# daisy9542/yolo-puncture

Hardware: AMD Instinct MI355X
Metric: images/sec (higher is better)
Workload: dtype bf16

## Files before the change

### include/yolop.h

```cpp
#ifndef YOLOP_H
#define YOLOP_H

#include <stddef.h>
#include <stdint.h>

#ifdef __cplusplus
extern "C" {
#endif

#define YP_OK 0
#define YP_ERR_ARG -1
#define YP_ERR_STATE -2
#define YP_ERR_HIP -3
#define YP_ERR_WEIGHT -4

#define YP_BF16 0
#define YP_F32 1

#define YP_TASK_DETECT 0
#define YP_TASK_SEGMENT 1

#define YP_NM 32
#define YP_MAX_MASKS 480
#define YP_ID_MASKS_FRAMES_BUDGET (1ull << 30)
// ... 124 lines not shown
int yp_tensor_read(yp_engine* e, int i, float* host_out);

int yp_profile(yp_engine* e, const uint8_t* in_dev, int B, int H, int W, float* det_out, int32_t* idx_out,
               float* coeff_out, float* ms_out, int iters, void* stream);

int yp_set_nms(yp_engine* e, float conf, float iou);

int yp_set_attention_form(yp_engine* e, int form);

int yp_set_autotune(yp_engine* e, int enable);

int yp_tuning_export(const yp_engine* e, int32_t* cfg_out, int cap);
int yp_tuning_import(yp_engine* e, int B, int H, int W, const int32_t* cfg, int n);

int yp_debug_force_conv_cfg(int cfg);
int yp_debug_op_cfg(const yp_engine* e, int i, int* cfg);
int yp_debug_last_store_form(void);
int yp_debug_max_workgroups(int n);
int yp_debug_conv_families(int* base, int* num_cfgs, int cap);
int yp_debug_ablation(int v);
int yp_debug_head_clocks(uint64_t* out8);
int yp_debug_attention(const void* qkv_dev, void* o_dev, int dtype, int B, int N, int nh, int kd, int hd, int q_stride, int q_coff, int o_stride,
                       int o_coff, int wgs, int* kernel_out, void* stream);
int yp_debug_attention_form(const void* qkv_dev, void* o_dev, int dtype, int B, int N, int nh, int kd, int hd, int q_stride, int q_coff, int o_stride,
                            int o_coff, int wgs, int form, int* kernel_out, void* stream);
int yp_debug_conv_s2(const void* x_dev, const void* w_dev, const float* bias_dev, const void* res_dev, void* y_dev, int out_f32, int B, int H,
                     int W, int Cin, int Cout, int silu, int cfg, int lds_weights, int64_t* lds_out, char* kernel_out, int kernel_cap,
                     void* stream);
int yp_debug_topk_anchors(const uint32_t* const mk_dev[3], int B, const int hw[3][2], int k, int32_t* sel_out_dev, uint32_t* thr_out_dev, void* stream);
int yp_debug_head_branch_clocks(uint64_t* out8);
int yp_debug_head_winners(yp_engine* e, int32_t* sel_host, float* box_host, float* coeff_host);
int yp_debug_contour_clocks(uint64_t* out12);
int yp_debug_pwsp_clocks(uint64_t* out32);

int yp_tuning_source(const yp_engine* e);

int yp_debug_host_selftest(yp_engine* e);
int yp_debug_graph_info(const yp_engine* e, int64_t* out6);
int yp_debug_head_positions(yp_engine* e, int64_t* out6);
int yp_debug_marker(void* stream);

int yp_set_graph(yp_engine* e, int enable);

#ifdef __cplusplus
}
#endif
#endif
```

### yolo-puncture_amd/csrc/common.h

```cpp
#pragma once
#include <hip/hip_runtime.h>
#include <stdint.h>
#include <atomic>
#include <cstdlib>
#include <string>
#include <vector>

namespace yp {

enum DType { DT_BF16 = 0, DT_F32 = 1 };
enum Act { ACT_NONE = 0, ACT_SILU = 1, ACT_RELU = 2 };

enum OpKind {
    OP_STEM = 0,
    OP_CONV = 1,
    OP_DWCONV = 2,
    OP_POOL5 = 3,
    OP_UPSAMPLE = 4,
    OP_ATTN = 5,
    OP_HEAD = 6,
    OP_CONVT = 7,
    OP_AMAX = 9,
    OP_POOL3 = 8,
};
// ... 319 lines not shown
hipError_t launch_anchor_max_level(const float* cls, int B, int HW, int nc, unsigned* out, hipStream_t st);

struct DwPwParams {
    const void* x; int x_stride, x_coff; int B, H, W, C; size_t x_bytes;
    const void* w_dw; const float* b_dw; int act_dw;
    const void* w_pw; int Kpad; size_t wpw_bytes; const float* b_pw; int act_pw;
    void* y; int y_stride, y_coff; size_t y_bytes; int Cout; int out_f32;
    unsigned long long* clk;
    int wide;
    const void* w3; int Kpad3; size_t w3_bytes; const float* b3; int C3;
    float* y3; int y3_stride, y3_coff; size_t y3_bytes;
    unsigned* keys;
};
bool dwpw_stream_valid(const DwPwParams& p);
hipError_t launch_dwpw_stream(const DwPwParams& p, hipStream_t st);
struct PwSpParams {
    const void* x; int x_stride, x_coff; size_t x_bytes; int B, H, W, K;
    const void* w1; const float* bias1; int act1, Kpad1, C1; size_t w1_bytes;
    void* y1; int y1_stride, y1_coff;
    const void* res1; int res1_stride, res1_coff;
    int sp;
    int sp_c0, Csp;
    const void* wd; const float* biasd; int actd;
    const void* res; int res_stride, res_coff;
    void* y2; int y2_stride, y2_coff;
    int dbg;
    int wide;
};
bool pwsp_valid(const PwSpParams& p);
const char* pwsp_kernel_name(const PwSpParams& p);
constexpr int PWSP_CFG = 1000;
hipError_t launch_pwsp(const PwSpParams& p, hipStream_t st);
hipError_t pwsp_read_clocks(unsigned long long* out32);

struct ClsOutParams {
    const void* x; int x_stride, x_coff; size_t x_bytes;
    int M, K, nc;
    const void* w; int Kpad; size_t w_bytes; const float* bias;
    float* y; int y_stride, y_coff;
    unsigned* keys;
};
bool cls_out_valid(const ClsOutParams& p);
const char* cls_out_kernel_name(const ClsOutParams& p);
hipError_t launch_cls_out(const ClsOutParams& p, hipStream_t st);

bool conv_dwpw_valid(const DwPwParams& p);
const char* conv_dwpw_kernel_name(const DwPwParams& p);
hipError_t launch_conv_dwpw(const DwPwParams& p, hipStream_t st);

struct MaskParams {
    const void* proto; int Hp, Wp;
    const float* coeff; const float* boxes; int n;
    int oh, ow;
    int t, l, ch, cw;
    float bsx, bsy;
    int crop_before;
    uint8_t* masks; int64_t* ids; int32_t* kept; int32_t* area;
    int suppress_small, min_area;
    int rh, rw;
};
hipError_t launch_masks(const MaskParams& p, int dtype, hipStream_t st);
size_t masks_workspace_bytes(const MaskParams& p);
struct MaskFramesParams {
    MaskParams p;
    const int32_t* fidx; int k;
    size_t proto_stride; long coeff_stride;
// ... 39 lines not shown
```

### yolo-puncture_amd/csrc/engine.hip

```cpp
#include "../../include/yolop.h"
#include "common.h"
#include <algorithm>
#include <array>
#include <chrono>

#include <cmath>
#include <cstdarg>
#include <cstdio>
#include <cstring>
#include <cstdlib>
#include <dlfcn.h>
#include <fcntl.h>
#include <fstream>
#include <map>
#include <sstream>
#include <memory>

using namespace yp;

static thread_local char g_err[512] = "";
static int fail(int code, const char* fmt, ...) {
    va_list ap;
    va_start(ap, fmt);
    vsnprintf(g_err, sizeof(g_err), fmt, ap);
// ... 2427 lines not shown
    if (!e->allocated) return fail(YP_ERR_STATE, "no forward has run yet");
    const Op* h = nullptr;
    for (const Op& o : e->ops) if (o.kind == OP_HEAD) h = &o;
    if (!h || !(h->sparse_box || h->sparse_cf) || !e->sp_ws) return 0;
    HIPCHK(hipSetDevice(e->device));
    HIPCHK(hipDeviceSynchronize());
    const SparseWs ws = sparse_ws_layout(*e);
    const char* base = (const char*)e->sp_ws;
    int pc[8];
    HIPCHK(hipMemcpy(pc, base + ws.pcount, sizeof(pc), hipMemcpyDeviceToHost));
    std::vector<int> wc((size_t)e->pB * 3);
    HIPCHK(hipMemcpy(wc.data(), base + ws.wcount, wc.size() * 4, hipMemcpyDeviceToHost));
    for (int l = 0; l < 3; ++l) {
        out6[l] = std::min(pc[4 + l], ws.plist_cap[l]);
        for (int b = 0; b < e->pB; ++b) out6[3 + l] += wc[(size_t)b * 3 + l];
    }
    return 1;
}

__global__ void op_marker_kernel(int* sink) { if (sink) *sink = 0; }
int yp_debug_marker(void* stream) {
    hipLaunchKernelGGL(op_marker_kernel, dim3(1), dim3(1), 0, (hipStream_t)stream, (int*)nullptr);
    HIPCHK(hipGetLastError());
    return YP_OK;
}

int yp_debug_pwsp_clocks(uint64_t* out32) {
    if (!out32) return fail(YP_ERR_ARG, "yp_debug_pwsp_clocks: null output");
    HIPCHK(hipDeviceSynchronize());
    HIPCHK(pwsp_read_clocks((unsigned long long*)out32));
    return YP_OK;
}

int yp_debug_contour_clocks(uint64_t* out12) {
    if (!out12) return fail(YP_ERR_ARG, "yp_debug_contour_clocks: null output");
    HIPCHK(hipDeviceSynchronize());
    HIPCHK(contour_read_clocks((unsigned long long*)out12));
    return YP_OK;
}

int yp_debug_ablation(int v) {
    conv_set_debug_ablation(v);
    return 0;
}

int yp_debug_force_conv_cfg(int cfg) {
    conv_dma_force_cfg(cfg);
    return conv_dma_family.num_cfgs;
}

int yp_debug_last_store_form(void) {
    store_form_watched().store(true);
    return last_store_form().exchange(-1);
}

int yp_debug_max_workgroups(int n) { return debug_max_workgroups_ref().exchange(n > 0 ? n : 0); }

int yp_debug_op_cfg(const yp_engine* e, int i, int* cfg) {
    if (!e || i < 0 || i >= (int)e->ops.size() || !cfg) return fail(YP_ERR_ARG, "bad argument");
    *cfg = op_launch_cfg(*e, e->ops[i]);
    return YP_OK;
}

int yp_debug_conv_families(int* base, int* num_cfgs, int cap) {
    for (int f = 0; f < kNumConvFamilies && f < cap; ++f) {
        if (base) base[f] = kConvFamilies[f]->base;
// ... 377 lines not shown
```

### yolo-puncture_amd/csrc/pwsp.hip

```cpp
#include "common.h"
#include <cstdlib>
#include <algorithm>

namespace yp {

typedef __attribute__((ext_vector_type(4))) unsigned u32x4;

__device__ unsigned long long g_ps_clk[32];
#define PS_STAMP(i) do { if (blockIdx.x == 0 && tid == 0) g_ps_clk[i] = __builtin_readcyclecounter(); } while (0)
hipError_t pwsp_read_clocks(unsigned long long* out32) { return hipMemcpyFromSymbol(out32, HIP_SYMBOL(g_ps_clk), 32 * sizeof(unsigned long long)); }

constexpr int PS_MF = 2;
constexpr int PS_NW = 16;
constexpr int PS_NT = PS_NW * 64;

template <int NS, int SP>
__global__ __launch_bounds__(PS_NT) void pwsp_kernel(const PwSpParams p) {
    constexpr int FN = NS / 16;
    constexpr int BK = 64, NSLOT = 3;
    constexpr int W_INSTR = NS / 8;
    constexpr int SLOT = W_INSTR * 1024;
    constexpr int KS = SP == 1 ? 3 : SP == 2 ? 7 : 1, PAD = KS / 2;
    constexpr int PIX = SP == 3 ? NS * 2 : NS * 2 + 8;
    constexpr int DW_NP = NS / 2, DW_G = PS_NT / DW_NP;
    constexpr int DW_PH = NS == 64 ? 5 : 3, DW_PW = 3;
    static_assert(SP != 3 || NS == 32, "the pool form keeps 64-byte pixel rows");

    extern __shared__ __attribute__((aligned(1024))) unsigned char smem[];
    unsigned char* const dump = smem + NSLOT * SLOT;
    unsigned char* const img = smem + NSLOT * SLOT + 1024;

    const int tid = threadIdx.x, lane = tid & 63;
    const int wave = __builtin_amdgcn_readfirstlane(tid >> 6);
    const int fr = lane & 15, fc = lane >> 4;
    const int HW = p.H * p.W;
    const int nsl = p.C1 / NS;
    const bool wide = SP == 0 && p.wide != 0;

    int b, sl;
    {
        const int bid = blockIdx.x, nwg = gridDim.x;
        if ((p.B & 7) == 0) { const int xcd = bid & 7, j = bid >> 3; b = (j / nsl) * 8 + xcd; sl = j % nsl; }
        else { b = bid / nsl; sl = bid % nsl; }
        (void)nwg;
    }
    PS_STAMP(0);
    const int n0 = sl * NS;
    const bool spatial = SP != 0 && n0 >= p.sp_c0 && n0 + NS <= p.sp_c0 + p.Csp;
    const int nk = (p.Kpad1 + BK - 1) / BK;
    const __amdgpu_buffer_rsrc_t wrs = __builtin_amdgcn_make_buffer_rsrc((void*)p.w1, 0, (int)p.w1_bytes, 0x00020000);

    const int dgx = (p.W + DW_PW - 1) / DW_PW, dgy = (p.H + DW_PH - 1) / DW_PH;
    const int IW = (SP == 1 || SP == 2) ? dgx * DW_PW + 2 * PAD : p.W, IH = (SP == 1 || SP == 2) ? dgy * DW_PH + 2 * PAD : p.H;
    constexpr int PXS = 256 * 128;
    unsigned char* const wring = smem;
    unsigned char* const pxa = img;
    unsigned char* const pxb = img + 2 * PXS;
    const int nmf = (HW + 15) >> 4;
    const __amdgpu_buffer_rsrc_t xrs = __builtin_amdgcn_make_buffer_rsrc((void*)p.x, 0, (int)p.x_bytes, 0x00020000);
    unsigned pa_off[2], pb_off[2];
    int p_kc[2], w_kc;
#pragma unroll
    for (int j = 0; j < 2; ++j) {
        const int row = (wave * 2 + j) * 8 + (lane >> 3);
        const int c = (lane & 7) ^ ((row >> 1) & 7);
        p_kc[j] = c * 8;
        pa_off[j] = (row < HW && row < 256) ? (unsigned)((b * HW + row) * p.x_stride + p.x_coff + c * 8) * 2u : kBufferOOB;
        pb_off[j] = (row + 256 < HW) ? (unsigned)((b * HW + row + 256) * p.x_stride + p.x_coff + c * 8) * 2u : kBufferOOB;
    }
    unsigned wconst;
    {
        const int s_ = wave * 64 + lane;
        const int row = s_ >> 3, pc = s_ & 7;
        const int c = pc ^ ((row >> 1) & 7);
        w_kc = c * 8;
        wconst = (wave < W_INSTR) ? (unsigned)(((n0 + weight_row_channel(row, wide)) * p.Kpad1 + c * 8) * 2) : kBufferOOB;
    }
    auto kbyte = [&](int kt) { return (unsigned)(kt * BK) * 2u; };
    auto issue_A = [&](int kt) {
        const bool live = kt < nk;
        const unsigned kb = kbyte(kt);
        __builtin_amdgcn_raw_ptr_buffer_load_lds(wrs, (lds_void*)((wave < W_INSTR) ? wring + (kt % NSLOT) * SLOT + wave * 1024 : dump), 16,
                                                 (live && wconst != kBufferOOB && kt * BK + w_kc < p.K) ? wconst + kb : kBufferOOB, 0, 0, 0);
#pragma unroll
        for (int j = 0; j < 2; ++j)
            __builtin_amdgcn_raw_ptr_buffer_load_lds(xrs, (lds_void*)(pxa + (kt & 1) * PXS + (wave * 2 + j) * 1024), 16,
                                                     (live && pa_off[j] != kBufferOOB && kt * BK + p_kc[j] < p.K && !(p.dbg & 2)) ? pa_off[j] + kb : kBufferOOB, 0, 0, 0);
    };
    auto issue_B = [&](int kt) {
        const bool live = kt < nk;
        const unsigned kb = kbyte(kt);
#pragma unroll
        for (int j = 0; j < 2; ++j)
            __builtin_amdgcn_raw_ptr_buffer_load_lds(xrs, (lds_void*)(pxb + (kt & 1) * PXS + (wave * 2 + j) * 1024), 16,
                                                     (live && pb_off[j] != kBufferOOB && kt * BK + p_kc[j] < p.K && !(p.dbg & 2)) ? pb_off[j] + kb : kBufferOOB, 0, 0, 0);
    };

    f32x4 acc[FN][PS_MF];
#pragma unroll
    for (int a = 0; a < FN; ++a) {
        const float4 b4 = *(const float4*)(p.bias1 + n0 + acc_channel(a, fc, wide));
#pragma unroll
        for (int f = 0; f < PS_MF; ++f) acc[a][f] = f32x4{b4.x, b4.y, b4.z, b4.w};
    }
    const bool hasA = wave < nmf, hasB = wave + 16 < nmf;
    issue_A(0); issue_B(0); issue_A(1);
    PS_STAMP(1);
    const unsigned fro = (unsigned)(fr * 128), frs = (unsigned)((fr >> 1) & 7);
    for (int g = 0; g < nk; ++g) {
        if (g < 16) PS_STAMP(8 + g);
        __builtin_amdgcn_s_waitcnt(5 | (7 << 4) | (0xF << 8));
        __builtin_amdgcn_s_barrier();
        issue_B(g + 1);
        const unsigned char* ws = wring + (g % NSLOT) * SLOT;
        bf16x8 wf[2][FN];
#pragma unroll
        for (int s_ = 0; s_ < 2; ++s_)
#pragma unroll
            for (int a = 0; a < FN; ++a) wf[s_][a] = *(const bf16x8*)(ws + a * 2048 + fro + (((unsigned)(s_ * 4 + fc) ^ frs) << 4));
        if (hasA && !(p.dbg & 1)) {
            const unsigned char* ps = pxa + (g & 1) * PXS + wave * 2048;
#pragma unroll
            for (int s_ = 0; s_ < 2; ++s_) {
                const bf16x8 xf = *(const bf16x8*)(ps + fro + (((unsigned)(s_ * 4 + fc) ^ frs) << 4));
#pragma unroll
                for (int a = 0; a < FN; ++a) acc[a][0] = __builtin_amdgcn_mfma_f32_16x16x32_bf16(wf[s_][a], xf, acc[a][0], 0, 0, 0);
            }
        }
        __builtin_amdgcn_s_waitcnt(5 | (7 << 4) | (0xF << 8));
        __builtin_amdgcn_s_barrier();
        issue_A(g + 2);
        if (hasB && !(p.dbg & 1)) {
            const unsigned char* ps = pxb + (g & 1) * PXS + wave * 2048;
#pragma unroll
            for (int s_ = 0; s_ < 2; ++s_) {
                const bf16x8 xf = *(const bf16x8*)(ps + fro + (((unsigned)(s_ * 4 + fc) ^ frs) << 4));
#pragma unroll
                for (int a = 0; a < FN; ++a) acc[a][1] = __builtin_amdgcn_mfma_f32_16x16x32_bf16(wf[s_][a], xf, acc[a][1], 0, 0, 0);
            }
        }
    }
    __builtin_amdgcn_s_waitcnt(0 | (7 << 4) | (0xF << 8));
    __syncthreads();
    if (SP == 1 || SP == 2) {
        if (spatial) {
            const int n16 = (IH * IW * PIX + 15) >> 4;
            for (int i = tid; i < n16; i += PS_NT) *(uint4*)(img + (size_t)i * 16) = make_uint4(0, 0, 0, 0);
            __syncthreads();
        }
    }

    PS_STAMP(2);
#pragma unroll
    for (int f = 0; f < PS_MF; ++f) {
        const int m = (wave + PS_NW * f) * 16 + fr;
        const bool ok = m < HW;
        const int py = ok ? m / p.W : 0, px = ok ? m - py * p.W : 0;
        if (wide) {
#pragma unroll
            for (int a = 0; a + 1 < FN; a += 2) {
                const int co = acc_channel(a, fc, true);
                float v[2][4];
#pragma unroll
                for (int h = 0; h < 2; ++h) {
#pragma unroll
                    for (int q = 0; q < 4; ++q) v[h][q] = acc[a + h][f][q];
                    if (p.act1 == ACT_SILU) silu4_packed(v[h]);
                }
                if (SP == 0 && p.res1) {
                    uint2 rr[2];
                    load_res_bf16x8((const __bf16*)p.res1 + (size_t)(b * HW + m) * p.res1_stride + p.res1_coff + n0 + co, ok, rr[0], rr[1]);
                    add_res_bf16x4(v[0], rr[0]);
                    add_res_bf16x4(v[1], rr[1]);
                }
                const u32x4 o = pack_bf16x8(v[0], v[1]);
                if (ok && p.y1) *(u32x4*)((__bf16*)p.y1 + (size_t)(b * HW + m) * p.y1_stride + p.y1_coff + n0 + co) = o;
            }
            continue;
        }
#pragma unroll
        for (int a = 0; a < FN; ++a) {
            float v[4] = {acc[a][f][0], acc[a][f][1], acc[a][f][2], acc[a][f][3]};
            if (p.act1 == ACT_SILU) silu4_packed(v);
            const int co = a * 16 + fc * 4;
            if (SP == 0 && p.res1 && ok) {
                const uint2 rr = *(const uint2*)((const __bf16*)p.res1 + (size_t)(b * HW + m) * p.res1_stride + p.res1_coff + n0 + co);
                add_res_bf16x4(v, rr);
            }
            const u32x2 o = pack_bf16x4(v);
            if (ok && p.y1) *(u32x2*)((__bf16*)p.y1 + (size_t)(b * HW + m) * p.y1_stride + p.y1_coff + n0 + co) = o;
            if (SP != 0 && ok && spatial) *(u32x2*)(img + (size_t)((py + PAD) * IW + px + PAD) * PIX + co * 2) = o;
        }
    }
    PS_STAMP(3);
    if (SP == 0) return;
    if (!spatial || (p.dbg & 4)) return;
    __syncthreads();
    PS_STAMP(4);

    const int cs0 = n0 - p.sp_c0;
    if constexpr (SP == 1 || SP == 2) {
        typedef __attribute__((address_space(3))) const unsigned* lds_u32p;
        typedef __attribute__((address_space(3))) const f32x2* lds_f2p;
        typedef __attribute__((address_space(3))) f32x2* lds_f2w;
        const int cp = tid % DW_NP, grp = tid / DW_NP;
        const int c = cs0 + cp * 2;
        const unsigned img_l = (unsigned)(size_t)(__attribute__((address_space(3))) unsigned char*)img;
        const unsigned wl_l = img_l + (unsigned)(((IH * IW * PIX) + 15) & ~15);
        f32x2 wk[KS == 3 ? 9 : 1];
        if constexpr (KS == 3) {
#pragma unroll
            for (int t = 0; t < 9; ++t) {
                const unsigned d = *(const unsigned*)((const __bf16*)p.wd + (size_t)t * p.Csp + c);
                wk[t] = f32x2{__uint_as_float(d << 16), __uint_as_float(d & 0xffff0000u)};
            }
        } else {
            for (int t = tid; t < KS * KS * DW_NP; t += PS_NT) {
// ... 70 lines not shown
            const unsigned char* src = (stage & 1) ? bufB : bufA;
            unsigned char* dst = (stage & 1) ? bufA : bufB;
            for (int i = tid; i < items; i += PS_NT) {
                const int pxl = i >> 2, y = pxl / W, x = pxl - y * W;
                const int x0 = max(x - 2, 0), x1 = max(x - 1, 0), x3 = min(x + 1, W - 1), x4 = min(x + 2, W - 1);
                const unsigned char* row = src + (size_t)(y * W) * 64 + (i & 3) * 16;
                uint4 m = *(const uint4*)(row + x * 64);
                m = pkmax4(m, *(const uint4*)(row + x0 * 64));
                m = pkmax4(m, *(const uint4*)(row + x1 * 64));
                m = pkmax4(m, *(const uint4*)(row + x3 * 64));
                m = pkmax4(m, *(const uint4*)(row + x4 * 64));
                *(uint4*)(tmp + i * 16) = m;
            }
            __syncthreads();
            __bf16* yb = (__bf16*)p.y2 + (size_t)b * HW * p.y2_stride + p.y2_coff + stage * p.Csp + cs0;
            for (int i = tid; i < items; i += PS_NT) {
                const int pxl = i >> 2, y = pxl / W, x = pxl - y * W;
                const int y0 = max(y - 2, 0), y1 = max(y - 1, 0), y3 = min(y + 1, H - 1), y4 = min(y + 2, H - 1);
                const unsigned char* col = tmp + (size_t)x * 64 + (i & 3) * 16;
                uint4 m = *(const uint4*)(col + (size_t)(y * W) * 64);
                m = pkmax4(m, *(const uint4*)(col + (size_t)(y0 * W) * 64));
                m = pkmax4(m, *(const uint4*)(col + (size_t)(y1 * W) * 64));
                m = pkmax4(m, *(const uint4*)(col + (size_t)(y3 * W) * 64));
                m = pkmax4(m, *(const uint4*)(col + (size_t)(y4 * W) * 64));
                *(uint4*)(dst + i * 16) = m;
                *(uint4*)(yb + (size_t)pxl * p.y2_stride + (i & 3) * 8) = bf16x8_key(m);
            }
            __syncthreads();
        }
    }
    PS_STAMP(5);
}

static size_t pwsp_lds_bytes(const PwSpParams& p, int NS) {
    const size_t ring = (size_t)3 * (NS / 8) * 1024 + 1024;
    const size_t px = (size_t)4 * 256 * 128;
    size_t sp = 0;
    if (p.sp == 3) sp = (size_t)p.H * p.W * 64 * 3;
    else if (p.sp != 0) {
        const int pad = p.sp == 1 ? 1 : 3, PH = NS == 64 ? 5 : 3, PW = 3;
        const int IH = (p.H + PH - 1) / PH * PH + 2 * pad, IW = (p.W + PW - 1) / PW * PW + 2 * pad;
        sp = (((size_t)IH * IW * (NS * 2 + 8) + 15) & ~(size_t)15) + (p.sp == 2 ? (size_t)49 * (NS / 2) * 8 : 0);
    }
    return ring + std::max(px, sp);
}

int pwsp_slice(const PwSpParams& p) {
    if (p.sp == 3) return 32;
    static const int force = env_int("YOLOP_PWSP_NS", 0);
    if (force == 32) return 32;
    if (force == 64 && (p.C1 % 64) == 0 && (p.sp == 0 || ((p.sp_c0 % 64) == 0 && (p.Csp % 64) == 0))) return 64;
    if ((p.C1 % 64) == 0 && (p.sp == 0 || ((p.sp_c0 % 64) == 0 && (p.Csp % 64) == 0)) && (long)p.B * (p.C1 / 64) >= 96) return 64;
    return 32;
}

bool pwsp_valid(const PwSpParams& p) {
    if (p.sp < 0 || p.sp > 3) return false;
    const int NS = pwsp_slice(p);
    if ((p.C1 % NS) != 0 || (p.K % 32) != 0 || p.Kpad1 != p.K || p.K < 64) return false;
    if (p.H * p.W > 16 * PS_MF * PS_NW || p.H < 1 || p.W < 1) return false;
    if ((p.x_stride & 7) || (p.x_coff & 7) || p.x_bytes >= (1ull << 31) || p.w1_bytes >= (1ull << 31)) return false;
    if (p.y1 && ((p.y1_stride & 3) || (p.y1_coff & 3))) return false;
    if (p.res1 && (p.sp != 0 || (p.res1_stride & 3) || (p.res1_coff & 3))) return false;
    if ((p.C1 + 127) / 128 * 128 < p.C1) return false;
    if (p.sp != 0) {
        if (!p.y2 || (p.sp_c0 % NS) != 0 || (p.Csp % NS) != 0 || p.sp_c0 < 0 || p.sp_c0 + p.Csp > p.C1) return false;
        if ((p.y2_stride & 7) || (p.y2_coff & 7)) return false;
        if (p.res && ((p.res_stride & 1) || (p.res_coff & 1))) return false;
        if (p.sp == 3 && p.res) return false;
    } else if (!p.y1) return false;
    return pwsp_lds_bytes(p, NS) <= 160 * 1024;
}

const char* pwsp_kernel_name(const PwSpParams& p) {
    const int NS = pwsp_slice(p);
    static const char* n[2][4] = {{"pwsp_kernel<32,0>", "pwsp_kernel<32,1>", "pwsp_kernel<32,2>", "pwsp_kernel<32,3>"},
                                  {"pwsp_kernel<64,0>", "pwsp_kernel<64,1>", "pwsp_kernel<64,2>", "pwsp_kernel<64,3>"}};
    return n[NS == 64][p.sp];
}

template <int NS, int SP>
static hipError_t launch_pwsp_t(const PwSpParams& p_in, hipStream_t st) {
    PwSpParams p = p_in;
    p.wide = (SP == 0 && p_in.y1 && wide_store_ok(p_in.wide, NS / 16, p_in.C1, p_in.y1_stride, p_in.y1_coff, false, p_in.res1, p_in.res1_stride, p_in.res1_coff)) ? 1 : 0;
    const size_t sh = pwsp_lds_bytes(p, NS);
    auto kern = pwsp_kernel<NS, SP>;
    static size_t granted = 0;
    if (hipError_t e = allow_dynamic_lds((const void*)kern, sh, granted)) return e;
    hipLaunchKernelGGL(kern, dim3((unsigned)(p.B * (p.C1 / NS))), dim3(PS_NT), sh, st, p);
    return hipGetLastError();
}

hipError_t launch_pwsp(const PwSpParams& p, hipStream_t st) {
    if (!pwsp_valid(p)) return hipErrorInvalidValue;
    const int NS = pwsp_slice(p);
    if (NS == 64) {
        switch (p.sp) {
            case 0: return launch_pwsp_t<64, 0>(p, st);
            case 1: return launch_pwsp_t<64, 1>(p, st);
            case 2: return launch_pwsp_t<64, 2>(p, st);
            default: return hipErrorInvalidValue;
        }
    }
    switch (p.sp) {
        case 0: return launch_pwsp_t<32, 0>(p, st);
        case 1: return launch_pwsp_t<32, 1>(p, st);
        case 2: return launch_pwsp_t<32, 2>(p, st);
        default: return launch_pwsp_t<32, 3>(p, st);
    }
}

}
```

### yolo-puncture_amd/engine.py

```python
from __future__ import annotations

import ctypes as C
import os
from typing import Dict, List, Optional, Tuple

import numpy as np
import torch

from .weights import fold_state

_LIB: Optional[C.CDLL] = None
_HERE = os.path.dirname(os.path.abspath(__file__))
LIB_PATH = os.environ.get("YOLOP_LIB") or os.path.join(_HERE, "libyolop.so")

YP_BF16, YP_F32 = 0, 1
TASK_DETECT, TASK_SEGMENT = 0, 1
OP_KINDS = {0: "stem", 1: "conv", 2: "dwconv", 3: "pool5", 4: "upsample", 5: "attn", 6: "head", 7: "convT", 8: "pool3", 9: "amax"}
FORMS = ("plain", "dwpw", "dwpw_tail", "s2pw", "frontend", "c2f", "scdown", "pwsp", "cls_out")


class ModelDesc(C.Structure):
    _fields_ = [("variant", C.c_int), ("nc", C.c_int), ("task", C.c_int), ("dtype", C.c_int), ("max_det", C.c_int), ("family", C.c_int)]


# ... 56 lines not shown
    lib.yp_tensor_write.argtypes = [vp, C.c_int, C.c_int, C.c_int, vp]
    lib.yp_tensor_count.argtypes = [vp]
    lib.yp_tensor_info.argtypes = [vp, C.c_int, C.c_char_p, C.c_int, ip, ip]
    lib.yp_tensor_read.argtypes = [vp, C.c_int, vp]
    lib.yp_profile.argtypes = [vp, vp, C.c_int, C.c_int, C.c_int, vp, vp, vp, vp, C.c_int, vp]
    lib.yp_set_graph.argtypes = [vp, C.c_int]
    lib.yp_set_autotune.argtypes = [vp, C.c_int]
    lib.yp_set_nms.argtypes = [vp, C.c_float, C.c_float]
    lib.yp_set_nms.restype = C.c_int
    lib.yp_debug_host_selftest.argtypes = [vp]
    lib.yp_debug_host_selftest.restype = C.c_int
    lib.yp_tuning_source.argtypes = [vp]
    lib.yp_tuning_source.restype = C.c_int
    lib.yp_debug_graph_info.argtypes = [vp, C.POINTER(C.c_int64)]
    lib.yp_debug_graph_info.restype = C.c_int
    lib.yp_debug_head_positions.argtypes = [vp, C.POINTER(C.c_int64)]
    lib.yp_debug_head_positions.restype = C.c_int
    lib.yp_debug_marker.argtypes = [vp]
    lib.yp_debug_marker.restype = C.c_int
    lib.yp_debug_force_conv_cfg.argtypes = [C.c_int]
    lib.yp_debug_op_cfg.argtypes = [vp, C.c_int, ip]
    lib.yp_debug_op_cfg.restype = C.c_int
    lib.yp_debug_last_store_form.argtypes = []
    lib.yp_debug_last_store_form.restype = C.c_int
    lib.yp_debug_max_workgroups.argtypes = [C.c_int]
    lib.yp_debug_max_workgroups.restype = C.c_int
    lib.yp_debug_conv_families.argtypes = [ip, ip, C.c_int]
    lib.yp_debug_conv_families.restype = C.c_int
    lib.yp_debug_ablation.argtypes = [C.c_int]
    lib.yp_debug_head_clocks.argtypes = [C.POINTER(C.c_uint64)]
    lib.yp_debug_head_branch_clocks.argtypes = [C.POINTER(C.c_uint64)]
    lib.yp_debug_contour_clocks.argtypes = [C.POINTER(C.c_uint64)]
    lib.yp_debug_pwsp_clocks.argtypes = [C.POINTER(C.c_uint64)]
    lib.yp_letterbox.argtypes = [vp, C.c_int, C.c_int, vp] + [C.c_int] * 7 + [vp]
    lib.yp_letterbox.restype = C.c_int
    lib.yp_letterbox_batch.argtypes = [vp, C.c_int, C.c_int, C.c_int, vp] + [C.c_int] * 7 + [vp]
    lib.yp_letterbox_batch.restype = C.c_int
    lib.yp_masks_frames.argtypes = [vp, vp, C.c_int, vp, C.c_long, vp, C.c_int, C.c_int, vp, vp]
    lib.yp_masks_frames.restype = C.c_int
    lib.yp_masks_frames_input.argtypes = [vp, vp, C.c_int, vp, C.c_long, vp, C.c_int, C.c_int, vp, vp]
    lib.yp_masks_frames_input.restype = C.c_int
    lib.yp_id_masks_frames.argtypes = [vp, vp, vp, C.c_int, vp, vp, C.c_int, C.c_int, C.c_int, C.c_int, vp, vp, C.c_int, C.c_int, vp]
    lib.yp_id_masks_frames.restype = C.c_int
    lib.yp_id_masks_frames_workspace.argtypes = [vp] + [C.c_int] * 6
    lib.yp_id_masks_frames_workspace.restype = C.c_size_t
    lib.yp_comm_unique_id.argtypes = [vp]
    lib.yp_comm_create.argtypes = [vp, C.c_int, C.c_int, C.c_int, C.POINTER(vp)]
    lib.yp_allgather.argtypes = [vp, vp, vp, C.c_size_t, vp]
    lib.yp_comm_destroy.argtypes = [vp]
    for fn in ("yp_comm_unique_id", "yp_comm_create", "yp_allgather", "yp_comm_destroy"):
        getattr(lib, fn).restype = C.c_int
    for fn in ("yp_create", "yp_destroy", "yp_weight_count", "yp_weight_info", "yp_set_weight", "yp_finalize",
               "yp_forward", "yp_proto", "yp_masks", "yp_plan", "yp_op_info", "yp_op_output", "yp_op_input", "yp_tensor_count",
               "yp_tensor_info", "yp_tensor_read", "yp_profile", "yp_set_graph", "yp_run_op", "yp_tensor_write",
               "yp_op_kernel", "yp_set_autotune", "yp_debug_force_conv_cfg", "yp_debug_ablation"):
        getattr(lib, fn).restype = C.c_int
    if path is None:
        _LIB = lib
    return lib


EXPORTS = ["yp_last_error", "yp_create", "yp_destroy", "yp_weight_count", "yp_weight_info", "yp_set_weight",
           "yp_finalize", "yp_forward", "yp_proto", "yp_masks", "yp_id_mask_resized", "yp_plan", "yp_op_info", "yp_op_output", "yp_op_input", "yp_op_fusion",
           "yp_tensor_count", "yp_tensor_info", "yp_tensor_read", "yp_profile", "yp_set_graph", "yp_run_op",
           "yp_tensor_write", "yp_op_kernel", "yp_set_autotune", "yp_tuning_export", "yp_tuning_import", "yp_set_nms", "yp_debug_force_conv_cfg", "yp_debug_op_cfg", "yp_debug_op_form", "yp_debug_last_store_form", "yp_debug_max_workgroups", "yp_debug_conv_families", "yp_debug_ablation", "yp_debug_head_clocks", "yp_debug_head_branch_clocks", "yp_debug_head_winners", "yp_debug_contour_clocks", "yp_debug_pwsp_clocks", "yp_debug_host_selftest", "yp_debug_graph_info", "yp_tuning_source", "yp_debug_head_positions", "yp_debug_marker", "yp_max_batch", "yp_debug_topk_anchors", "yp_debug_attention", "yp_debug_attention_form", "yp_debug_conv_s2", "yp_set_attention_form", "yp_letterbox", "yp_letterbox_batch", "yp_masks_frames", "yp_masks_frames_input", "yp_id_masks_frames", "yp_id_masks_frames_workspace", "yp_mask_contours",
           "yp_mask_contours_scaled", "yp_mask_contours_large_workspace", "yp_mask_contours_large", "yp_comm_unique_id", "yp_comm_create", "yp_allgather", "yp_comm_destroy",
           "yp_u2net_create", "yp_u2net_destroy", "yp_u2net_weight_count", "yp_u2net_weight_info", "yp_u2net_set_weight", "yp_u2net_finalize",
           "yp_u2net_forward", "yp_u2net_forward_crops", "yp_u2net_set_graph", "yp_u2net_tensor_count", "yp_u2net_tensor_info", "yp_u2net_tensor_read",
           "yp_u2net_op_count", "yp_u2net_op_info",
           "yp_cls_create", "yp_cls_destroy", "yp_cls_weight_count", "yp_cls_weight_info", "yp_cls_set_weight", "yp_cls_finalize",
           "yp_cls_forward", "yp_cls_set_graph", "yp_cls_tensor_count", "yp_cls_tensor_info", "yp_cls_tensor_read"]


MAX_ANCHORS = 294912
MAX_MASKS = 480
ID_MASKS_FRAMES_BUDGET = 1 << 30
ATTENTION_FORMS = {"auto": 0, "stream": 1, "stream_wide": 3}


def _attention_form(form) -> int:
    if form not in ATTENTION_FORMS:
        raise ValueError(f"attention form {form!r}: one of {sorted(ATTENTION_FORMS)}")
    return ATTENTION_FORMS[form]


def topk_anchors(mk: List[torch.Tensor], hw, k: int) -> Tuple[torch.Tensor, torch.Tensor]:
    lib = load_library()
    if len(mk) != 3 or len(hw) != 3:
        raise ValueError("three levels")
    B = int(mk[0].shape[0])
    dev = mk[0].device
    for t, (h, w) in zip(mk, hw):
        if t.dtype != torch.int32 or not t.is_contiguous() or t.device != dev or tuple(t.shape) != (B, int(h) * int(w)):
            raise ValueError("mk[l] must be contiguous int32 [B, H_l * W_l] on one device")
    sel = torch.full((B, 512), -1, dtype=torch.int32, device=dev)
    thr = torch.zeros((B,), dtype=torch.int32, device=dev)
    ptrs = (C.c_void_p * 3)(*[t.data_ptr() for t in mk])
    hwa = (C.c_int * 6)(*[int(v) for pair in hw for v in pair])
# ... 517 lines not shown
```

Before: 23600.

## Split pwsp GEMM loop into producer loader waves and MFMA consumer waves

Adds a warp-specialized main loop to the fused pointwise+spatial kernel: 8 waves only issue buffer-to-LDS loads while 8 waves run the MFMA loop with hand-scheduled ds_read and lgkmcnt waits, each holding four M fragments. This is meant to overlap global loads with matrix math instead of having every wave do both in lock-step. The new path is the default, selected through YOLOP_PWSP_LOOP, and a debug entry point can force either loop. It raises accumulator register pressure per compute wave and leaves half the waves without MFMA work.

```diff
diff --git a/include/yolop.h b/include/yolop.h
--- a/include/yolop.h
+++ b/include/yolop.h
@@ -180,6 +180,7 @@
 int yp_debug_head_winners(yp_engine* e, int32_t* sel_host, float* box_host, float* coeff_host);
 int yp_debug_contour_clocks(uint64_t* out12);
 int yp_debug_pwsp_clocks(uint64_t* out32);
+int yp_debug_pwsp_loop(int loop);
 
 int yp_tuning_source(const yp_engine* e);
 
diff --git a/yolo-puncture_amd/csrc/common.h b/yolo-puncture_amd/csrc/common.h
--- a/yolo-puncture_amd/csrc/common.h
+++ b/yolo-puncture_amd/csrc/common.h
@@ -375,6 +375,7 @@
 constexpr int PWSP_CFG = 1000;
 hipError_t launch_pwsp(const PwSpParams& p, hipStream_t st);
 hipError_t pwsp_read_clocks(unsigned long long* out32);
+bool pwsp_debug_loop(int v);
 
 struct ClsOutParams {
     const void* x; int x_stride, x_coff; size_t x_bytes;
diff --git a/yolo-puncture_amd/csrc/engine.hip b/yolo-puncture_amd/csrc/engine.hip
--- a/yolo-puncture_amd/csrc/engine.hip
+++ b/yolo-puncture_amd/csrc/engine.hip
@@ -2483,6 +2483,11 @@
     return YP_OK;
 }
 
+int yp_debug_pwsp_loop(int loop) {
+    if (!pwsp_debug_loop(loop)) return fail(YP_ERR_ARG, "yp_debug_pwsp_loop: %d is no loop (-1 default, 0 lock-step, 1 split)", loop);
+    return YP_OK;
+}
+
 int yp_debug_contour_clocks(uint64_t* out12) {
     if (!out12) return fail(YP_ERR_ARG, "yp_debug_contour_clocks: null output");
     HIPCHK(hipDeviceSynchronize());
diff --git a/yolo-puncture_amd/csrc/pwsp.hip b/yolo-puncture_amd/csrc/pwsp.hip
--- a/yolo-puncture_amd/csrc/pwsp.hip
+++ b/yolo-puncture_amd/csrc/pwsp.hip
@@ -1,6 +1,8 @@
 #include "common.h"
 #include <cstdlib>
 #include <algorithm>
+#include <atomic>
+#include <type_traits>
 
 namespace yp {
 
@@ -13,10 +15,28 @@
 constexpr int PS_MF = 2;
 constexpr int PS_NW = 16;
 constexpr int PS_NT = PS_NW * 64;
-
-template <int NS, int SP>
-__global__ __launch_bounds__(PS_NT) void pwsp_kernel(const PwSpParams p) {
+constexpr int PS_NC = 8;
+
+template <int OFF> __device__ __forceinline__ void ps_rd(bf16x8& d, unsigned addr) {
+    static_assert(OFF >= 0 && OFF < 65536, "ds offset field");
+    asm volatile("ds_read_b128 %0, %1 offset:%2" : "=v"(d) : "v"(addr), "n"(OFF));
+}
+template <int N> __device__ __forceinline__ void ps_wait(bf16x8& x) {
+    static_assert(N >= 0 && N < 16, "lgkmcnt range");
+    asm volatile("s_waitcnt lgkmcnt(%1)" : "+v"(x) : "n"(N) : "memory");
+}
+template <int N, int FN> __device__ __forceinline__ void ps_wait(bf16x8 (&w)[FN], bf16x8& x) {
+    static_assert(N >= 0 && N < 16, "lgkmcnt range");
+    static_assert(FN == 2 || FN == 4, "operand list of the wait");
+    if constexpr (FN == 4) asm volatile("s_waitcnt lgkmcnt(%5)" : "+v"(w[0]), "+v"(w[1]), "+v"(w[2]), "+v"(w[3]), "+v"(x) : "n"(N) : "memory");
+    else asm volatile("s_waitcnt lgkmcnt(%3)" : "+v"(w[0]), "+v"(w[1]), "+v"(x) : "n"(N) : "memory");
+}
+
+template <int NS, int SP, int LOOP>
+__device__ __forceinline__ void pwsp_body(const PwSpParams& p) {
     constexpr int FN = NS / 16;
+    constexpr int MF = LOOP ? 32 / PS_NC : PS_MF;
+    constexpr int FS = LOOP ? PS_NC : PS_NW;
     constexpr int BK = 64, NSLOT = 3;
     constexpr int W_INSTR = NS / 8;
     constexpr int SLOT = W_INSTR * 1024;
@@ -58,6 +78,22 @@
     unsigned char* const pxb = img + 2 * PXS;
     const int nmf = (HW + 15) >> 4;
     const __amdgpu_buffer_rsrc_t xrs = __builtin_amdgcn_make_buffer_rsrc((void*)p.x, 0, (int)p.x_bytes, 0x00020000);
+    auto kbyte = [&](int kt) { return (unsigned)(kt * BK) * 2u; };
+    const unsigned fro = (unsigned)(fr * 128), frs = (unsigned)((fr >> 1) & 7);
+    const bool has_acc = LOOP == 0 || wave < PS_NC;
+    f32x4 acc[FN][MF];
+    auto acc_bias = [&]() {
+#pragma unroll
+        for (int a = 0; a < FN; ++a) {
+            int co = acc_channel(a, fc, wide);
+            if constexpr (LOOP != 0) asm volatile("" : "+v"(co));
+            const float4 b4 = *(const float4*)(p.bias1 + n0 + co);
+#pragma unroll
+            for (int f = 0; f < MF; ++f) acc[a][f] = f32x4{b4.x, b4.y, b4.z, b4.w};
+        }
+    };
+    if constexpr (LOOP == 0) acc_bias();
+    if constexpr (LOOP == 0) {
     unsigned pa_off[2], pb_off[2];
     int p_kc[2], w_kc;
 #pragma unroll
@@ -76,7 +112,6 @@
         w_kc = c * 8;
         wconst = (wave < W_INSTR) ? (unsigned)(((n0 + weight_row_channel(row, wide)) * p.Kpad1 + c * 8) * 2) : kBufferOOB;
     }
-    auto kbyte = [&](int kt) { return (unsigned)(kt * BK) * 2u; };
     auto issue_A = [&](int kt) {
         const bool live = kt < nk;
         const unsigned kb = kbyte(kt);
@@ -96,17 +131,9 @@
                                                      (live && pb_off[j] != kBufferOOB && kt * BK + p_kc[j] < p.K && !(p.dbg & 2)) ? pb_off[j] + kb : kBufferOOB, 0, 0, 0);
     };
 
-    f32x4 acc[FN][PS_MF];
-#pragma unroll
-    for (int a = 0; a < FN; ++a) {
-        const float4 b4 = *(const float4*)(p.bias1 + n0 + acc_channel(a, fc, wide));
-#pragma unroll
-        for (int f = 0; f < PS_MF; ++f) acc[a][f] = f32x4{b4.x, b4.y, b4.z, b4.w};
-    }
     const bool hasA = wave < nmf, hasB = wave + 16 < nmf;
     issue_A(0); issue_B(0); issue_A(1);
     PS_STAMP(1);
-    const unsigned fro = (unsigned)(fr * 128), frs = (unsigned)((fr >> 1) & 7);
     for (int g = 0; g < nk; ++g) {
         if (g < 16) PS_STAMP(8 + g);
         __builtin_amdgcn_s_waitcnt(5 | (7 << 4) | (0xF << 8));
@@ -140,6 +167,129 @@
             }
         }
     }
+    } else if (wave >= PS_NC) {
+        constexpr int LP = 32 / PS_NC;
+        const int l = wave - PS_NC;
+        unsigned la_off[LP], lb_off[LP], lw_off;
+        int l_kc[LP], lw_kc;
+#pragma unroll
+        for (int j = 0; j < LP; ++j) {
+            const int row = (l * LP + j) * 8 + (lane >> 3);
+            const int c = (lane & 7) ^ ((row >> 1) & 7);
+            l_kc[j] = c * 8;
+            la_off[j] = (row < HW) ? (unsigned)((b * HW + row) * p.x_stride + p.x_coff + c * 8) * 2u : kBufferOOB;
+            lb_off[j] = (row + 256 < HW) ? (unsigned)((b * HW + row + 256) * p.x_stride + p.x_coff + c * 8) * 2u : kBufferOOB;
+        }
+        {
+            const int row = l * 8 + (lane >> 3), pc = lane & 7;
+            const int c = pc ^ ((row >> 1) & 7);
+            lw_kc = c * 8;
+            lw_off = (l < W_INSTR) ? (unsigned)(((n0 + weight_row_channel(row, wide)) * p.Kpad1 + c * 8) * 2) : kBufferOOB;
+        }
+        auto issue_A = [&](int kt) {
+            const bool live = kt < nk;
+            const unsigned kb = kbyte(kt);
+            __builtin_amdgcn_raw_ptr_buffer_load_lds(wrs, (lds_void*)((l < W_INSTR) ? wring + (kt % NSLOT) * SLOT + l * 1024 : dump), 16,
+                                                     (live && lw_off != kBufferOOB && kt * BK + lw_kc < p.K) ? lw_off + kb : kBufferOOB, 0, 0, 0);
+#pragma unroll
+            for (int j = 0; j < LP; ++j)
+                __builtin_amdgcn_raw_ptr_buffer_load_lds(xrs, (lds_void*)(pxa + (kt & 1) * PXS + (l * LP + j) * 1024), 16,
+                                                         (live && la_off[j] != kBufferOOB && kt * BK + l_kc[j] < p.K && !(p.dbg & 2)) ? la_off[j] + kb : kBufferOOB, 0, 0, 0);
+        };
+        auto issue_B = [&](int kt) {
+            const bool live = kt < nk;
+            const unsigned kb = kbyte(kt);
+#pragma unroll
+            for (int j = 0; j < LP; ++j)
+                __builtin_amdgcn_raw_ptr_buffer_load_lds(xrs, (lds_void*)(pxb + (kt & 1) * PXS + (l * LP + j) * 1024), 16,
+                                                         (live && lb_off[j] != kBufferOOB && kt * BK + l_kc[j] < p.K && !(p.dbg & 2)) ? lb_off[j] + kb : kBufferOOB, 0, 0, 0);
+        };
+        issue_A(0); issue_B(0); issue_A(1);
+        for (int g = 0; g < nk; ++g) {
+            wait_vmcnt<2 * LP + 1>();
+            __builtin_amdgcn_s_barrier();
+            issue_B(g + 1);
+            wait_vmcnt<2 * LP + 1>();
+            __builtin_amdgcn_s_barrier();
+            issue_A(g + 2);
+        }
+    } else {
+        const int c = wave;
+        const bool mm = !(p.dbg & 1);
+        const int nA = mm ? (c < nmf) + (c + 8 < nmf) : 0, nB = mm ? (c + 16 < nmf) + (c + 24 < nmf) : 0;
+        const unsigned xo0 = fro + ((((unsigned)fc) ^ frs) << 4), xo1 = fro + ((((unsigned)(4 + fc)) ^ frs) << 4);
+        const unsigned w_l = lds_addr(wring), a_l = lds_addr(pxa) + (unsigned)(c * 2048), b_l = lds_addr(pxb) + (unsigned)(c * 2048);
+        bf16x8 wf[2][FN];
+        auto rd_w = [](bf16x8 (&w)[FN], unsigned addr) {
+            ps_rd<0>(w[0], addr); ps_rd<2048>(w[1], addr);
+            if constexpr (FN == 4) { ps_rd<4096>(w[2], addr); ps_rd<6144>(w[3], addr); }
+        };
+        auto mm_frag = [&](bf16x8 (&w)[FN], const bf16x8& x, auto f_) {
+            constexpr int f = decltype(f_)::value;
+#pragma unroll
+            for (int a = 0; a < FN; ++a) acc[a][f] = __builtin_amdgcn_mfma_f32_16x16x32_bf16(w[a], x, acc[a][f], 0, 0, 0);
+        };
+        using std::integral_constant;
+        auto phase_a = [&](auto nf_, unsigned wb, unsigned xb) {
+            constexpr int NF = decltype(nf_)::value;
+            bf16x8 x0, x1, y0, y1;
+            rd_w(wf[0], wb + xo0); ps_rd<0>(x0, xb + xo0); if constexpr (NF == 2) ps_rd<8 * 2048>(x1, xb + xo0);
+            rd_w(wf[1], wb + xo1);
+            ps_wait<FN + NF - 1, FN>(wf[0], x0);
+            mm_frag(wf[0], x0, integral_constant<int, 0>{});
+            __builtin_amdgcn_sched_barrier(0);
+            ps_rd<0>(y0, xb + xo1);
+            if constexpr (NF == 2) {
+                ps_wait<FN + 1>(x1);
+                mm_frag(wf[0], x1, integral_constant<int, 1>{});
+                __builtin_amdgcn_sched_barrier(0);
+                ps_rd<8 * 2048>(y1, xb + xo1);
+            }
+            ps_wait<NF - 1, FN>(wf[1], y0);
+            mm_frag(wf[1], y0, integral_constant<int, 0>{});
+            if constexpr (NF == 2) { __builtin_amdgcn_sched_barrier(0); ps_wait<0>(y1); mm_frag(wf[1], y1, integral_constant<int, 1>{}); }
+            __builtin_amdgcn_sched_barrier(0);
+        };
+        auto phase_b = [&](auto nf_, unsigned xb) {
+            constexpr int NF = decltype(nf_)::value;
+            bf16x8 x0, x1, y0, y1;
+            ps_rd<0>(x0, xb + xo0); if constexpr (NF == 2) ps_rd<8 * 2048>(x1, xb + xo0);
+            ps_wait<NF - 1>(x0);
+            mm_frag(wf[0], x0, integral_constant<int, 2>{});
+            __builtin_amdgcn_sched_barrier(0);
+            ps_rd<0>(y0, xb + xo1);
+            if constexpr (NF == 2) {
+                ps_wait<1>(x1);
+                mm_frag(wf[0], x1, integral_constant<int, 3>{});
+                __builtin_amdgcn_sched_barrier(0);
+                ps_rd<8 * 2048>(y1, xb + xo1);
+            }
+            ps_wait<NF - 1>(y0);
+            mm_frag(wf[1], y0, integral_constant<int, 2>{});
+            if constexpr (NF == 2) { __builtin_amdgcn_sched_barrier(0); ps_wait<0>(y1); mm_frag(wf[1], y1, integral_constant<int, 3>{}); }
+            __builtin_amdgcn_sched_barrier(0);
+        };
+        PS_STAMP(1);
+        auto k_loop = [&](auto na_, auto nb_) {
+            acc_bias();
+#pragma unroll
+            for (int a = 0; a < FN; ++a) asm volatile("" : "+v"(acc[a][0]), "+v"(acc[a][1]), "+v"(acc[a][2]), "+v"(acc[a][3]));
+            for (int g = 0; g < nk; ++g) {
+                if (g < 16) PS_STAMP(8 + g);
+                __builtin_amdgcn_s_barrier();
+                const unsigned wb = w_l + (unsigned)((g % NSLOT) * SLOT), po = (unsigned)((g & 1) * PXS);
+                if constexpr (decltype(na_)::value > 0) phase_a(na_, wb, a_l + po);
+                __builtin_amdgcn_s_barrier();
+                if constexpr (decltype(nb_)::value > 0) phase_b(nb_, b_l + po);
+            }
+        };
+        const integral_constant<int, 0> i0; const integral_constant<int, 1> i1; const integral_constant<int, 2> i2;
+        if (nB == 2) k_loop(i2, i2);
+        else if (nB == 1) k_loop(i2, i1);
+        else if (nA == 2) k_loop(i2, i0);
+        else if (nA == 1) k_loop(i1, i0);
+        else k_loop(i0, i0);
+    }
     __builtin_amdgcn_s_waitcnt(0 | (7 << 4) | (0xF << 8));
     __syncthreads();
     if (SP == 1 || SP == 2) {
@@ -151,15 +301,19 @@
     }
 
     PS_STAMP(2);
-#pragma unroll
-    for (int f = 0; f < PS_MF; ++f) {
-        const int m = (wave + PS_NW * f) * 16 + fr;
+    int lane_e = lane;
+#pragma unroll
+    for (int f = 0; f < MF; ++f) {
+        if (!has_acc || (LOOP != 0 && wave + FS * f >= nmf)) continue;
+        if constexpr (LOOP != 0) asm volatile("" : "+v"(lane_e));
+        const int fr_e = lane_e & 15, fc_e = lane_e >> 4;
+        const int m = (wave + FS * f) * 16 + fr_e;
         const bool ok = m < HW;
         const int py = ok ? m / p.W : 0, px = ok ? m - py * p.W : 0;
         if (wide) {
 #pragma unroll
             for (int a = 0; a + 1 < FN; a += 2) {
-                const int co = acc_channel(a, fc, true);
+                const int co = acc_channel(a, fc_e, true);
                 float v[2][4];
 #pragma unroll
                 for (int h = 0; h < 2; ++h) {
@@ -182,7 +336,7 @@
         for (int a = 0; a < FN; ++a) {
             float v[4] = {acc[a][f][0], acc[a][f][1], acc[a][f][2], acc[a][f][3]};
             if (p.act1 == ACT_SILU) silu4_packed(v);
-            const int co = a * 16 + fc * 4;
+            const int co = a * 16 + fc_e * 4;
             if (SP == 0 && p.res1 && ok) {
                 const uint2 rr = *(const uint2*)((const __bf16*)p.res1 + (size_t)(b * HW + m) * p.res1_stride + p.res1_coff + n0 + co);
                 add_res_bf16x4(v, rr);
@@ -319,6 +473,26 @@
     PS_STAMP(5);
 }
 
+template <int NS, int SP>
+__global__ __launch_bounds__(PS_NT) void pwsp_kernel(const PwSpParams p) { pwsp_body<NS, SP, 1>(p); }
+template <int NS, int SP, int LOOP>
+__global__ __launch_bounds__(PS_NT) void pwsp_kernel(const PwSpParams p) {
+    static_assert(LOOP == 0, "the third argument is the lock-step loop");
+    pwsp_body<NS, SP, LOOP>(p);
+}
+
+static std::atomic<int>& pwsp_loop_ref() {
+    static std::atomic<int> v{env_int("YOLOP_PWSP_LOOP", 1) != 0 ? 1 : 0};
+    return v;
+}
+static std::atomic<int> g_pwsp_loop_forced{-1};
+bool pwsp_debug_loop(int v) {
+    if (v < -1 || v > 1) return false;
+    g_pwsp_loop_forced.store(v);
+    return true;
+}
+static int pwsp_loop() { const int f = g_pwsp_loop_forced.load(); return f >= 0 ? f : pwsp_loop_ref().load(); }
+
 static size_t pwsp_lds_bytes(const PwSpParams& p, int NS) {
     const size_t ring = (size_t)3 * (NS / 8) * 1024 + 1024;
     const size_t px = (size_t)4 * 256 * 128;
@@ -371,9 +545,10 @@
     PwSpParams p = p_in;
     p.wide = (SP == 0 && p_in.y1 && wide_store_ok(p_in.wide, NS / 16, p_in.C1, p_in.y1_stride, p_in.y1_coff, false, p_in.res1, p_in.res1_stride, p_in.res1_coff)) ? 1 : 0;
     const size_t sh = pwsp_lds_bytes(p, NS);
-    auto kern = pwsp_kernel<NS, SP>;
-    static size_t granted = 0;
-    if (hipError_t e = allow_dynamic_lds((const void*)kern, sh, granted)) return e;
+    const int loop = pwsp_loop();
+    void (*const kern)(const PwSpParams) = loop ? pwsp_kernel<NS, SP> : pwsp_kernel<NS, SP, 0>;
+    static size_t granted[2] = {0, 0};
+    if (hipError_t e = allow_dynamic_lds((const void*)kern, sh, granted[loop])) return e;
     hipLaunchKernelGGL(kern, dim3((unsigned)(p.B * (p.C1 / NS))), dim3(PS_NT), sh, st, p);
     return hipGetLastError();
 }
diff --git a/yolo-puncture_amd/engine.py b/yolo-puncture_amd/engine.py
--- a/yolo-puncture_amd/engine.py
+++ b/yolo-puncture_amd/engine.py
@@ -112,6 +112,8 @@
     lib.yp_debug_head_branch_clocks.argtypes = [C.POINTER(C.c_uint64)]
     lib.yp_debug_contour_clocks.argtypes = [C.POINTER(C.c_uint64)]
     lib.yp_debug_pwsp_clocks.argtypes = [C.POINTER(C.c_uint64)]
+    lib.yp_debug_pwsp_loop.argtypes = [C.c_int]
+    lib.yp_debug_pwsp_loop.restype = C.c_int
     lib.yp_letterbox.argtypes = [vp, C.c_int, C.c_int, vp] + [C.c_int] * 7 + [vp]
     lib.yp_letterbox.restype = C.c_int
     lib.yp_letterbox_batch.argtypes = [vp, C.c_int, C.c_int, C.c_int, vp] + [C.c_int] * 7 + [vp]
@@ -143,7 +145,7 @@
 EXPORTS = ["yp_last_error", "yp_create", "yp_destroy", "yp_weight_count", "yp_weight_info", "yp_set_weight",
            "yp_finalize", "yp_forward", "yp_proto", "yp_masks", "yp_id_mask_resized", "yp_plan", "yp_op_info", "yp_op_output", "yp_op_input", "yp_op_fusion",
            "yp_tensor_count", "yp_tensor_info", "yp_tensor_read", "yp_profile", "yp_set_graph", "yp_run_op",
-           "yp_tensor_write", "yp_op_kernel", "yp_set_autotune", "yp_tuning_export", "yp_tuning_import", "yp_set_nms", "yp_debug_force_conv_cfg", "yp_debug_op_cfg", "yp_debug_op_form", "yp_debug_last_store_form", "yp_debug_max_workgroups", "yp_debug_conv_families", "yp_debug_ablation", "yp_debug_head_clocks", "yp_debug_head_branch_clocks", "yp_debug_head_winners", "yp_debug_contour_clocks", "yp_debug_pwsp_clocks", "yp_debug_host_selftest", "yp_debug_graph_info", "yp_tuning_source", "yp_debug_head_positions", "yp_debug_marker", "yp_max_batch", "yp_debug_topk_anchors", "yp_debug_attention", "yp_debug_attention_form", "yp_debug_conv_s2", "yp_set_attention_form", "yp_letterbox", "yp_letterbox_batch", "yp_masks_frames", "yp_masks_frames_input", "yp_id_masks_frames", "yp_id_masks_frames_workspace", "yp_mask_contours",
+           "yp_tensor_write", "yp_op_kernel", "yp_set_autotune", "yp_tuning_export", "yp_tuning_import", "yp_set_nms", "yp_debug_force_conv_cfg", "yp_debug_op_cfg", "yp_debug_op_form", "yp_debug_last_store_form", "yp_debug_max_workgroups", "yp_debug_conv_families", "yp_debug_ablation", "yp_debug_head_clocks", "yp_debug_head_branch_clocks", "yp_debug_head_winners", "yp_debug_contour_clocks", "yp_debug_pwsp_clocks", "yp_debug_pwsp_loop", "yp_debug_host_selftest", "yp_debug_graph_info", "yp_tuning_source", "yp_debug_head_positions", "yp_debug_marker", "yp_max_batch", "yp_debug_topk_anchors", "yp_debug_attention", "yp_debug_attention_form", "yp_debug_conv_s2", "yp_set_attention_form", "yp_letterbox", "yp_letterbox_batch", "yp_masks_frames", "yp_masks_frames_input", "yp_id_masks_frames", "yp_id_masks_frames_workspace", "yp_mask_contours",
            "yp_mask_contours_scaled", "yp_mask_contours_large_workspace", "yp_mask_contours_large", "yp_comm_unique_id", "yp_comm_create", "yp_allgather", "yp_comm_destroy",
            "yp_u2net_create", "yp_u2net_destroy", "yp_u2net_weight_count", "yp_u2net_weight_info", "yp_u2net_set_weight", "yp_u2net_finalize",
            "yp_u2net_forward", "yp_u2net_forward_crops", "yp_u2net_set_graph", "yp_u2net_tensor_count", "yp_u2net_tensor_info", "yp_u2net_tensor_read",
```

Measured after the change: 23790 (median of 6 runs). About the same (+0.8%).
